# xhuan8/SoccerPlayerShapePose

Hardware: NVIDIA B200
Metric: SMPL meshes/sec fwd+bwd (higher is better)
Workload: dtype f32 (bf16x3 split on tcgen05, fp32 accumulate)

## Files before the change

### soccerplayershapepose_b200/build.py

```python
from __future__ import annotations

import concurrent.futures
import os
import shutil
import subprocess
import sys

HERE = os.path.dirname(os.path.abspath(__file__))
CSRC = os.path.join(HERE, "csrc")
BUILD = os.path.join(HERE, "csrc", "build")
LIB = os.path.join(HERE, "libb200smpl.so")

SOURCES = ["api.cu", "pack.cu", "pose.cu", "blend_simt.cu", "blend_umma.cu", "fused_fwd.cu", "lbs.cu", "joints.cu", "aux_ops.cu", "fit.cu", "loss.cu", "silhouette.cu"]
HEADERS = [os.path.join(CSRC, h) for h in sorted(os.listdir(CSRC)) if h.endswith(".cuh")] + [
    os.path.join(HERE, "..", "include", "b200smpl.h")]

NVCC_FLAGS = [
    "-gencode", "arch=compute_100a,code=sm_100a",
    "-O3", "-std=c++17", "-lineinfo",
    "-Xcompiler", "-fPIC",
    "-Xcompiler", "-fvisibility=hidden",
    "--expt-relaxed-constexpr",
    "-Xptxas", "-v",
]


def _nvcc() -> str:
    for cand in (os.environ.get("NVCC"), "/usr/local/cuda/bin/nvcc", shutil.which("nvcc")):
        if cand and os.path.exists(cand):
            return cand
    raise RuntimeError("nvcc not found (needed to build libb200smpl.so)")


def _stale(target: str, deps) -> bool:
    if not os.path.exists(target):
        return True
# ... 45 lines not shown
```

### soccerplayershapepose_b200/csrc/api.cu

```cuda
#include <atomic>
#include <cstring>
#include <map>
#include <mutex>

#include <nvtx3/nvToolsExt.h>

#include "common.cuh"
#include "umma_common.cuh"

namespace b200smpl {

bool pdl_enabled() {
  static const bool on = getenv("B200_PDL") == nullptr || atoi(getenv("B200_PDL")) != 0;
  return on;
}

NvtxRange::NvtxRange(const char* name) { nvtxRangePushA(name); }
NvtxRange::~NvtxRange() { nvtxRangePop(); }

static thread_local std::string g_last_error;
static std::atomic<long long> g_launches{0};

void set_error(const std::string& msg) { g_last_error = msg; }
int fail(int code, const std::string& msg) {
// ... 50 lines not shown
  const int S = slab_bodies > 0 ? round_up(std::min(slab_bodies, MAX_SLAB), 128) : DEFAULT_SLAB;
  p.S = std::min(S, Bp);
  size_t off = 0;
  auto take = [&](size_t bytes) {
    const size_t o = off;
    off = align_up(off + bytes, 1024);
    return o;
  };
  const size_t S_ = (size_t)p.S;
  p.off_feat = take(S_ * d.fl.pitch * 2);
  p.off_featf = take(mode == B200SMPL_MODE_FP32_SIMT ? S_ * d.fl.nf_pad * 4 : 0);
  p.off_A = take((size_t)NJ * AELEMS * S_ * 4);
  p.off_jposed = take((size_t)NJ * 3 * S_ * 4);
  p.off_vpT = take((size_t)d.n_pad * S_ * 4);
  p.saved_slab_bytes = align_up((size_t)NJ * AELEMS * S_ * 4, 1024) + align_up((size_t)d.n_pad * S_ * 4, 1024);
  if (backward) {
    const int bmode = bwd_gemm_mode(mode);
    p.k_splits = bmode == B200SMPL_MODE_FP32_SIMT ? 1 : blend_bwd_umma_splits(d, p.S, m->num_sms);
    p.off_dvp_hi = take(S_ * d.n_pad * 2);
    p.off_dvp_lo = take(bmode == B200SMPL_MODE_BF16 ? 0 : S_ * d.n_pad * 2);
    p.off_dA = take((size_t)(NJ * AELEMS + 3) * S_ * 4);
    p.off_dtr = p.off_dA + (size_t)NJ * AELEMS * S_ * 4;
    p.off_dJtot = take((size_t)std::max(batch, 1) * d.njout * 3 * 4);
    p.off_dfeat = take((size_t)p.k_splits * S_ * d.fl.nf_pad * 4);
  }
  p.total = off + 1024;
  return p;
}

static int check_common(const b200smpl_model* m, int batch, int mode, const void* ws) {
  if (m == nullptr) return fail(B200SMPL_ERR_INVALID, "null model handle");
  if (m->device < 0) return fail(B200SMPL_ERR_CUDA, "host-only model handle: no CUDA device (there is no CPU fallback)");
  if (batch < 1) return fail(B200SMPL_ERR_INVALID, "batch must be >= 1");
  if (mode != B200SMPL_MODE_FP32 && mode != B200SMPL_MODE_BF16 && mode != B200SMPL_MODE_FP32_SIMT &&
      mode != B200SMPL_MODE_BF16_FAST)
    return fail(B200SMPL_ERR_INVALID, "unknown mode");
  if (ws == nullptr) return fail(B200SMPL_ERR_WORKSPACE, "null workspace");
  return 0;
}

}

using namespace b200smpl;

extern "C" {

int b200smpl_abi_version(void) { return B200SMPL_ABI_VERSION; }
// ... 63 lines not shown
    m->num_sms = prop.multiProcessorCount;
    if (prop.major != 10) {
      cleanup();
      cudaSetDevice(prev);
      return fail(B200SMPL_ERR_CUDA, "this library is built for sm_100a (B200) only; device is sm_" +
                                         std::to_string(prop.major) + std::to_string(prop.minor));
    }
  }
  auto upload = [&](const void* src, size_t bytes, const void** dst) -> bool {
    void* p = nullptr;
    if (cudaMalloc(&p, std::max<size_t>(bytes, 16)) != cudaSuccess) return false;
    m->allocs.push_back(p);
    if (bytes && cudaMemcpy(p, src, bytes, cudaMemcpyHostToDevice) != cudaSuccess) return false;
    *dst = p;
    return true;
  };
  HostArrays& h = m->host;
  DevModel& d = m->dm;
  bool ok = true;
#define UP(field, vec) ok = ok && upload((vec).data(), (vec).size() * sizeof((vec)[0]), (const void**)&d.field)
  UP(Wf, h.Wf);
  UP(Wb_hi, h.Wb_hi);
  UP(Wb_lo, h.Wb_lo);
  UP(W32, h.W32);
  UP(vmeta, h.vmeta);
  UP(vwts, h.vwts);
  UP(vplan, h.vplan);
  UP(Jt, h.Jt);
  UP(Jsd, h.Jsd);
  UP(term_ptr, h.term_ptr);
  UP(term_joint, h.term_joint);
  UP(term_qrow, h.term_qrow);
  UP(term_c, h.term_c);
  UP(qmeta, h.qmeta);
  UP(qcoef, h.qcoef);
  UP(vt_j0, h.vt_j0);
  UP(vt_nj, h.vt_nj);
#undef UP
  cudaSetDevice(prev);
  if (!ok) {
    e = cudaGetLastError();
    cleanup();
    return fail(B200SMPL_ERR_CUDA, std::string("model upload failed: ") + cudaGetErrorString(e));
  }
  *out = m;
  return 0;
// ... 163 lines not shown
    const int nb = std::min(S, B - b0);
    const int Sw = round_up(nb, 128);
    B200_CUDA_TRY(cudaMemsetAsync(dA_part, 0, (size_t)(NJ * AELEMS + 3) * S * 4, st));
    if (saved) {
      A_T = (float*)(saved + (size_t)(b0 / S) * p.saved_slab_bytes);
      vpT = (float*)((char*)A_T + align_up((size_t)NJ * AELEMS * S * 4, 1024));
    } else {
      if ((rc = launch_pose_fwd(d, a->betas, a->pose, aa, b0, nb, S, Sw, feat, featf, A_T, nullptr, nullptr, st)))
        return rc;
      if (a->mode == B200SMPL_MODE_FP32_SIMT)
        rc = launch_blend_fwd_simt(d, featf, S, Sw, vpT, row_begin, d.n_pad, st);
      else
        rc = launch_blend_fwd_umma(d, fwd_gemm_mode(a->mode), feat, S, Sw, vpT, row_begin, d.n_pad, m->num_sms, st);
      if (rc) return rc;
    }
    {
      const size_t c0 = (size_t)row_end / 8, c1 = (size_t)round_up(row_end, 64) / 8;
      if (c1 > c0) {
        const size_t pitch = (size_t)(d.n_pad / 8) * 2048, width = (c1 - c0) * 2048;
        B200_CUDA_TRY(cudaMemset2DAsync(dvp_hi + c0 * 1024, pitch, 0, width, (size_t)Sw / 128, st));
        if (dvp_lo) B200_CUDA_TRY(cudaMemset2DAsync(dvp_lo + c0 * 1024, pitch, 0, width, (size_t)Sw / 128, st));
      }
    }
    if (have_v)
      if ((rc = launch_lbs_bwd(d, vpT, S, Sw, A_T, b0, nb, a->grad_vertices, dvp_hi, dvp_lo, dA_part, dtr_part,
                               m->num_sms, st)))
        return rc;
    if (have_j)
      if ((rc = launch_joints_bwd(d, vpT, S, Sw, A_T, b0, nb, dJ, dvp_hi, dvp_lo, dA_part, dtr_part, have_v, st))) return rc;
    if (a->mode == B200SMPL_MODE_FP32_SIMT)
      rc = launch_blend_bwd_simt(d, dvp_hi, dvp_lo, S, Sw, dfeat_part, row_begin, row_end, st);
    else
      rc = launch_blend_bwd_umma(d, bmode, dvp_hi, dvp_lo, S, Sw, dfeat_part, k_splits, row_begin, row_end, st);
    if (rc) return rc;
    if ((rc = launch_pose_bwd(d, a->betas, a->pose, aa, b0, nb, S, A_T, dA_part, 1, dtr_part, dfeat_part, k_splits,
                              have_j ? dJ : nullptr, a->grad_betas, a->grad_pose, a->grad_transl, st)))
      return rc;
  }
  return 0;
}

}
```

### soccerplayershapepose_b200/csrc/common.cuh

```cuda
#pragma once

#include <cuda_bf16.h>
#include <cuda_runtime.h>
#include <stdint.h>

#include <cstring>
#include <string>
#include <utility>
#include <vector>

#include "../../include/b200smpl.h"

namespace b200smpl {

constexpr int NJ = 24;
constexpr int NPOSE = 9 * (NJ - 1);
constexpr int AELEMS = 12;
constexpr int TILE_V = 32;
constexpr int MAX_CHILD = 4;
constexpr int MAX_BETAS = 16;

constexpr uint32_t VMETA_VALID = 1u << 29;

struct ChainTables {
// ... 34 lines not shown
  L.pitch = 64 + 2 * L.pseg;
  L.nf = nb + NPOSE;
  L.nf_pad = round_up(L.nf, 16);
  return L;
}

struct DevModel {
  int V;
  int ntiles;
  int n_real;
  int nq;
  int n_rows;
  int n_virt0;
  int n_pad;
  int njout;
  int nterms;
  int ntv;
  int vt_maxcols;
  FeatLayout fl;
  ChainTables chain;
  const __nv_bfloat16* Wf;
  const __nv_bfloat16* Wb_hi;
  const __nv_bfloat16* Wb_lo;
  const float* W32;
  const uint32_t* vmeta;
  const float4* vwts;
  const uint32_t* vplan;
  const float* Jt;
  const float* Jsd;
  const int32_t* term_ptr;
  const uint8_t* term_joint;
  const int32_t* term_qrow;
  const float* term_c;
  const uint32_t* qmeta;
  const float* qcoef;
  const int32_t* vt_j0;
  const int32_t* vt_nj;
};

struct HostArrays {
  std::vector<__nv_bfloat16> Wf, Wb_hi, Wb_lo;
  std::vector<float> W32, Jt, Jsd, term_c;
  std::vector<uint32_t> vmeta;
  std::vector<float> vwts;
  std::vector<uint32_t> vplan;
  std::vector<int32_t> term_ptr, term_qrow, vt_j0, vt_nj;
  std::vector<int8_t> chain_order, chain_level_ptr;
  std::vector<uint32_t> qmeta;
  std::vector<float> qcoef;
  std::vector<uint8_t> term_joint;
};

}

struct b200smpl_model {
  int device = -1;
  b200smpl::DevModel dm{};
  b200smpl::HostArrays host;
  std::vector<void*> allocs;
  int nvj = 0, nreg = 0;
  int num_sms = 148;
};

namespace b200smpl {
// ... 66 lines not shown
    ::b200smpl::count_launch();                                                                   \
  } while (0)

int pack_model(const b200smpl_model_desc* d, HostArrays& h, DevModel& dm, std::string& err);

int launch_pose_fwd(const DevModel& m, const float* betas, const float* pose, bool axis_angle, int b0, int nb, int S,
                    int Sw, __nv_bfloat16* feat, float* featf, float* A_blk, const float* transl, float* joints,
                    cudaStream_t st);
int launch_pose_bwd(const DevModel& m, const float* betas, const float* pose, bool axis_angle, int b0, int nb, int S,
                    const float* A_blk, const float* dA_part, int n_dA_parts, const float* dtr_part, const float* dfeat_part,
                    int n_dfeat_parts, const float* dJ, float* grad_betas, float* grad_pose,
                    float* grad_transl, cudaStream_t st);

int launch_blend_fwd_simt(const DevModel& m, const float* featf, int S, int Sw, float* vpT, int row_begin,
                          int row_end, cudaStream_t st);
int launch_blend_bwd_simt(const DevModel& m, const __nv_bfloat16* dvp_hi, const __nv_bfloat16* dvp_lo, int S, int Sw,
                          float* dfeat, int row_begin, int row_end, cudaStream_t st);
int launch_blend_fwd_umma(const DevModel& m, int mode, const __nv_bfloat16* feat, int S, int Sw, float* vpT,
                          int row_begin, int row_end, int num_sms, cudaStream_t st);
int launch_blend_bwd_umma(const DevModel& m, int mode, const __nv_bfloat16* dvp_hi, const __nv_bfloat16* dvp_lo,
                          int S, int Sw, float* dfeat_part, int nsplit, int row_begin, int row_end,
                          cudaStream_t st);
int blend_bwd_umma_splits(const DevModel& m, int S, int num_sms);
int launch_blend_lbs_fwd(const DevModel& m, int mode, const __nv_bfloat16* feat, int S, int Sw, float* vpT,
                         const float* A_blk, int b0, int nb, const float* transl, float* verts, int num_sms,
                         cudaStream_t st);

int launch_lbs_fwd(const DevModel& m, const float* vpT, int S, const float* A_T, int b0, int nb,
                   const float* transl, float* verts, int num_sms, cudaStream_t st);
int launch_lbs_bwd(const DevModel& m, const float* vpT, int S, int Sw, const float* A_T, int b0, int nb,
                   const float* grad_verts, __nv_bfloat16* dvp_hi, __nv_bfloat16* dvp_lo, float* dA_acc,
                   float* dtr_acc, int num_sms, cudaStream_t st);

int launch_joints_fwd(const DevModel& m, const float* vpB, int S, const float* A_blk, int b0, int nb,
                      const float* transl, float* joints, bool after_lbs, cudaStream_t st);
int launch_joints_bwd(const DevModel& m, const float* vpB, int S, int Sw, const float* A_blk, int b0, int nb,
                      const float* dJ, __nv_bfloat16* dvp_hi, __nv_bfloat16* dvp_lo, float* dA_part, float* dtr_part,
                      bool after_lbs, cudaStream_t st);
int launch_joint_grad_total(const float* joints, const float* cam, const float* gj, const float* g2d, float* dJ,
                            float* gcam, int B, int nj, cudaStream_t st);

}
```

### soccerplayershapepose_b200/csrc/lbs.cu

```cuda
#include "lbs_tiles.cuh"

namespace b200smpl {


struct CtaRange {
  int begin, end;
};
__device__ __forceinline__ CtaRange make_cta_range(int ngroups, int nitems) {
  const long long total = (long long)ngroups * nitems;
  CtaRange r;
  r.begin = (int)(total * blockIdx.x / gridDim.x);
  r.end = (int)(total * (blockIdx.x + 1) / gridDim.x);
  return r;
}

template <int HV>
__device__ __forceinline__ void issue_item(float4* vbuf, uint32_t* stash, uint64_t* bar, const float4* __restrict__ vp_group,
                                           const uint32_t* __restrict__ vplan, int t) {
  using SH = ItemShape<HV>;
  mbar_expect_tx(bar, SH::TX_BYTES);
  bulk_g2s(vbuf, vp_group + (size_t)t * (SH::NCH4 * 32), SH::VP_WORDS * 4, bar);
  bulk_g2s(stash, vplan + (size_t)t * SH::PLAN_WORDS, SH::PLAN_WORDS * 4, bar);
}
template <int HV>
__device__ __forceinline__ void global_to_tile_scalar(float* tile, const float* src0, size_t row_stride, int nrows,
                                                      int ncols, int lane) {
  for (int r = 0; r < 32; ++r)
    for (int c = lane; c < ItemShape<HV>::ROWS; c += 32)
      tile[r * ItemShape<HV>::HROW + c] = (r < nrows && c < ncols) ? src0[(size_t)r * row_stride + c] : 0.f;
}

constexpr int FWD_RUN = 1;
constexpr int FWD_HV = 16;
constexpr int FWD_WARPS = 8;
constexpr int FWD_THREADS = FWD_WARPS * 32;
constexpr int FWD_WARP_WORDS = ItemShape<FWD_HV>::TILE_WORDS + 2 * (ItemShape<FWD_HV>::VP_WORDS + ItemShape<FWD_HV>::PLAN_WORDS) + 4;
constexpr size_t FWD_SMEM = (size_t)(AG_WORDS + FWD_WARPS * FWD_WARP_WORDS) * 4 + 16;

template <bool HI>
__device__ __forceinline__ void load_slot2(SlotXY& s, SlotZ2& z, const float* A_s, int joint, int lane) {
  const float4* p = reinterpret_cast<const float4*>(A_s) + joint * 96 + lane;
  const float4 q0 = p[0], q1 = p[32], q2 = p[64];
  s.c0 = mk2(q0.x, q0.y); s.c1 = mk2(q0.z, q0.w); s.c2 = mk2(q1.x, q1.y); s.t = mk2(q1.z, q1.w);
  z.r20 = set_half<HI>(z.r20, q2.x); z.r21 = set_half<HI>(z.r21, q2.y);
  z.r22 = set_half<HI>(z.r22, q2.z); z.t2 = set_half<HI>(z.t2, q2.w);
}
// ... 347 lines not shown
```

### soccerplayershapepose_b200/csrc/lbs_tiles.cuh

```cuda
#pragma once

#include "skin_common.cuh"

namespace b200smpl {

template <int HV>
struct ItemShape {
  static constexpr int ROWS = HV * 3;
  static constexpr int HROW = ROWS + 4;
  static constexpr int TILE_WORDS = 32 * HROW;
  static constexpr int NCH4 = ROWS / 4;
  static constexpr int NCH8 = ROWS / 8;
  static constexpr int PAIRS = ROWS / 2;
  static constexpr int VP_WORDS = NCH4 * 128;
  static constexpr int PLAN_WORDS = (HV / 8) * 40;
  static constexpr uint32_t TX_BYTES = (VP_WORDS + PLAN_WORDS) * 4;
  static_assert((HROW / 4) % 2 == 1 && ROWS % 8 == 0 && HV % 8 == 0, "item shape");
};

__device__ __forceinline__ const float4* plan_wts(const uint32_t* stash, int u) {
  return reinterpret_cast<const float4*>(stash + (u >> 1) * 40 + (u & 1) * 16);
}
__device__ __forceinline__ const uint32_t* plan_meta(const uint32_t* stash, int u) {
  return stash + (u >> 1) * 40 + 32 + (u & 1) * 4;
}

template <int HV>
__device__ __forceinline__ void tile_to_global_full(const float* tile, float* dst0, size_t row_stride, int lane) {
  using SH = ItemShape<HV>;
  constexpr int RPP = 96 / SH::PAIRS, J = 32 / RPP;
  float* gp[3];
  const float* sp[3];
#pragma unroll
  for (int kk = 0; kk < 3; ++kk) {
    const int piece = kk * 32 + lane, rr = piece / SH::PAIRS, c = (piece - rr * SH::PAIRS) * 2;
    gp[kk] = dst0 + (size_t)rr * row_stride + c;
    sp[kk] = tile + rr * SH::HROW + c;
  }
  const size_t step = (size_t)RPP * row_stride;
#pragma unroll
  for (int j = 0; j < J; ++j)
#pragma unroll
// ... 120 lines not shown
```

### soccerplayershapepose_b200/csrc/pack.cu

```cuda
#include <algorithm>
#include <array>
#include <cmath>
#include <cstring>
#include <map>
#include <numeric>

#include "common.cuh"

namespace b200smpl {

static inline __nv_bfloat16 h_bf16(float x) { return __float2bfloat16_rn(x); }
static inline float h_f32(__nv_bfloat16 x) { return __bfloat162float(x); }

int pack_model(const b200smpl_model_desc* d, HostArrays& h, DevModel& dm, std::string& err) {
  const int V = d->num_verts, nb = d->num_betas, nvj = d->num_vertex_joints, nreg = d->num_regressed_joints;
  if (d->num_joints != NJ) { err = "num_joints must be 24"; return B200SMPL_ERR_INVALID; }
  if (V < 1 || V > (1 << 20)) { err = "bad num_verts"; return B200SMPL_ERR_INVALID; }
  if (nb < 1 || nb > MAX_BETAS) { err = "num_betas must be in [1,16]"; return B200SMPL_ERR_INVALID; }
  if (!d->v_template || !d->shapedirs || !d->posedirs || !d->J_regressor || !d->lbs_weights || !d->parents ||
      (nvj > 0 && !d->vertex_joint_ids) || (nreg > 0 && !d->joint_regressors)) {
    err = "null model array";
    return B200SMPL_ERR_INVALID;
  }
  const FeatLayout fl = make_feat_layout(nb);
// ... 163 lines not shown
  h.Wb_hi.assign((size_t)fl.nf_pad * n_pad, h_bf16(0.f));
  h.Wb_lo.assign((size_t)fl.nf_pad * n_pad, h_bf16(0.f));
  for (int n = 0; n < n_rows; ++n) {
    __nv_bfloat16* wr = h.Wf.data() + (size_t)n * fl.pitch;
    {
      const float t = h.W32[n];
      const __nv_bfloat16 t0 = h_bf16(t);
      const __nv_bfloat16 t1 = h_bf16(t - h_f32(t0));
      const __nv_bfloat16 t2 = h_bf16(t - h_f32(t0) - h_f32(t1));
      wr[0] = t0; wr[1] = t1; wr[2] = t2;
    }
    for (int f = 0; f < nf; ++f) {
      const float x = h.W32[(size_t)(1 + f) * n_pad + n];
      const __nv_bfloat16 hi = h_bf16(x), lo = h_bf16(x - h_f32(hi));
      if (f < nb) {
        wr[fl.off_s0 + f] = hi; wr[fl.off_s1 + f] = hi; wr[fl.off_s2 + f] = lo;
      } else {
        const int p = f - nb;
        wr[fl.off_p0 + p] = hi; wr[fl.off_p1 + p] = lo;
      }
      h.Wb_hi[(size_t)f * n_pad + n] = hi;
      h.Wb_lo[(size_t)f * n_pad + n] = lo;
    }
  }

  h.Jt.assign(NJ * 3, 0.f);
  h.Jsd.assign((size_t)NJ * 3 * nb, 0.f);
  for (int j = 0; j < NJ; ++j) {
    std::vector<double> acc(3 * (1 + nb), 0.0);
    for (int v = 0; v < V; ++v) {
      const double r = d->J_regressor[(size_t)j * V + v];
      if (r == 0.0) continue;
      for (int k = 0; k < 3; ++k) {
        acc[k * (1 + nb)] += r * (double)d->v_template[v * 3 + k];
        for (int l = 0; l < nb; ++l) acc[k * (1 + nb) + 1 + l] += r * (double)d->shapedirs[((size_t)v * 3 + k) * nb + l];
      }
    }
    for (int k = 0; k < 3; ++k) {
      h.Jt[j * 3 + k] = (float)acc[k * (1 + nb)];
      for (int l = 0; l < nb; ++l) h.Jsd[((size_t)j * 3 + k) * nb + l] = (float)acc[k * (1 + nb) + 1 + l];
    }
  }

  h.vmeta.assign((size_t)ntiles * TILE_V, 0u);
  h.vwts.assign((size_t)ntiles * TILE_V * 4, 0.f);
  {
// ... 76 lines not shown
```

Before: 6.913 million.

## Fuse LBS backward with blend-shape backward GEMM in a 2-CTA tcgen05 kernel

Adds a clustered 2-CTA kernel that computes the skinning backward (dA, dtrans) and writes the per-vertex position gradients straight into tensor memory as the A operand of a tcgen05 GEMM against a reinterleaved blend-weight matrix. This produces the dfeat partials without materializing dvp_hi/dvp_lo in global memory. The host gains a new interleaved weight layout and a work list, and the fused path only handles vertex gradients, so joint gradients still take the old blend backward path over the virtual rows. This trades two kernels and the global round trip of dvp for a heavier warp-specialized kernel with more partial slots to reduce.

```diff
diff --git a/soccerplayershapepose_b200/build.py b/soccerplayershapepose_b200/build.py
--- a/soccerplayershapepose_b200/build.py
+++ b/soccerplayershapepose_b200/build.py
@@ -11,7 +11,7 @@
 BUILD = os.path.join(HERE, "csrc", "build")
 LIB = os.path.join(HERE, "libb200smpl.so")
 
-SOURCES = ["api.cu", "pack.cu", "pose.cu", "blend_simt.cu", "blend_umma.cu", "fused_fwd.cu", "lbs.cu", "joints.cu", "aux_ops.cu", "fit.cu", "loss.cu", "silhouette.cu"]
+SOURCES = ["api.cu", "pack.cu", "pose.cu", "blend_simt.cu", "blend_umma.cu", "fused_fwd.cu", "fused_bwd.cu", "lbs.cu", "joints.cu", "aux_ops.cu", "fit.cu", "loss.cu", "silhouette.cu"]
 HEADERS = [os.path.join(CSRC, h) for h in sorted(os.listdir(CSRC)) if h.endswith(".cuh")] + [
     os.path.join(HERE, "..", "include", "b200smpl.h")]
 
diff --git a/soccerplayershapepose_b200/csrc/api.cu b/soccerplayershapepose_b200/csrc/api.cu
--- a/soccerplayershapepose_b200/csrc/api.cu
+++ b/soccerplayershapepose_b200/csrc/api.cu
@@ -96,7 +96,9 @@
     p.off_dA = take((size_t)(NJ * AELEMS + 3) * S_ * 4);
     p.off_dtr = p.off_dA + (size_t)NJ * AELEMS * S_ * 4;
     p.off_dJtot = take((size_t)std::max(batch, 1) * d.njout * 3 * 4);
-    p.off_dfeat = take((size_t)p.k_splits * S_ * d.fl.nf_pad * 4);
+    int parts = p.k_splits;
+    if (bmode != B200SMPL_MODE_FP32_SIMT) parts = std::max(0, fused_bwd_parts(d, p.S, m->num_sms)) + p.k_splits;
+    p.off_dfeat = take((size_t)parts * S_ * d.fl.nf_pad * 4);
   }
   p.total = off + 1024;
   return p;
@@ -206,6 +208,8 @@
   UP(Wf, h.Wf);
   UP(Wb_hi, h.Wb_hi);
   UP(Wb_lo, h.Wb_lo);
+  UP(Wbi_hi, h.Wbi_hi);
+  UP(Wbi_lo, h.Wbi_lo);
   UP(W32, h.W32);
   UP(vmeta, h.vmeta);
   UP(vwts, h.vwts);
@@ -415,18 +419,38 @@
         if (dvp_lo) B200_CUDA_TRY(cudaMemset2DAsync(dvp_lo + c0 * 1024, pitch, 0, width, (size_t)Sw / 128, st));
       }
     }
-    if (have_v)
-      if ((rc = launch_lbs_bwd(d, vpT, S, Sw, A_T, b0, nb, a->grad_vertices, dvp_hi, dvp_lo, dA_part, dtr_part,
-                               m->num_sms, st)))
+    int n_parts = k_splits;
+    if (have_v && fused_bwd_usable(d, a->mode, a->grad_vertices)) {
+      const int nfp = fused_bwd_parts(d, Sw, m->num_sms);
+      if (nfp < 0) return fail(B200SMPL_ERR_INVALID, "slab too wide for the fused backward work list");
+      B200_CUDA_TRY(cudaMemsetAsync(dfeat_part, 0, (size_t)nfp * S * d.fl.nf_pad * 4, st));
+      if ((rc = launch_lbs_bwd_gemm(d, bmode, vpT, S, Sw, A_T, b0, nb, a->grad_vertices, dA_part, dtr_part, dfeat_part,
+                                    m->num_sms, st)))
         return rc;
-    if (have_j)
-      if ((rc = launch_joints_bwd(d, vpT, S, Sw, A_T, b0, nb, dJ, dvp_hi, dvp_lo, dA_part, dtr_part, have_v, st))) return rc;
-    if (a->mode == B200SMPL_MODE_FP32_SIMT)
-      rc = launch_blend_bwd_simt(d, dvp_hi, dvp_lo, S, Sw, dfeat_part, row_begin, row_end, st);
-    else
-      rc = launch_blend_bwd_umma(d, bmode, dvp_hi, dvp_lo, S, Sw, dfeat_part, k_splits, row_begin, row_end, st);
-    if (rc) return rc;
-    if ((rc = launch_pose_bwd(d, a->betas, a->pose, aa, b0, nb, S, A_T, dA_part, 1, dtr_part, dfeat_part, k_splits,
+      n_parts = nfp;
+      if (have_j) {
+        if ((rc = launch_joints_bwd(d, vpT, S, Sw, A_T, b0, nb, dJ, dvp_hi, dvp_lo, dA_part, dtr_part, false, st))) return rc;
+        const int vslabs = (row_end + 63) / 64 - d.n_virt0 / 64;
+        const int ksv = std::max(1, std::min(p.k_splits, vslabs / MIN_SLABS_PER_SPLIT));
+        if ((rc = launch_blend_bwd_umma(d, bmode, dvp_hi, dvp_lo, S, Sw, dfeat_part + (size_t)nfp * S * d.fl.nf_pad, ksv,
+                                        d.n_virt0, row_end, st)))
+          return rc;
+        n_parts += ksv;
+      }
+    } else {
+      if (have_v)
+        if ((rc = launch_lbs_bwd(d, vpT, S, Sw, A_T, b0, nb, a->grad_vertices, dvp_hi, dvp_lo, dA_part, dtr_part,
+                                 m->num_sms, st)))
+          return rc;
+      if (have_j)
+        if ((rc = launch_joints_bwd(d, vpT, S, Sw, A_T, b0, nb, dJ, dvp_hi, dvp_lo, dA_part, dtr_part, have_v, st))) return rc;
+      if (a->mode == B200SMPL_MODE_FP32_SIMT)
+        rc = launch_blend_bwd_simt(d, dvp_hi, dvp_lo, S, Sw, dfeat_part, row_begin, row_end, st);
+      else
+        rc = launch_blend_bwd_umma(d, bmode, dvp_hi, dvp_lo, S, Sw, dfeat_part, k_splits, row_begin, row_end, st);
+      if (rc) return rc;
+    }
+    if ((rc = launch_pose_bwd(d, a->betas, a->pose, aa, b0, nb, S, A_T, dA_part, 1, dtr_part, dfeat_part, n_parts,
                               have_j ? dJ : nullptr, a->grad_betas, a->grad_pose, a->grad_transl, st)))
       return rc;
   }
diff --git a/soccerplayershapepose_b200/csrc/common.cuh b/soccerplayershapepose_b200/csrc/common.cuh
--- a/soccerplayershapepose_b200/csrc/common.cuh
+++ b/soccerplayershapepose_b200/csrc/common.cuh
@@ -80,6 +80,8 @@
   const __nv_bfloat16* Wf;
   const __nv_bfloat16* Wb_hi;
   const __nv_bfloat16* Wb_lo;
+  const __nv_bfloat16* Wbi_hi;
+  const __nv_bfloat16* Wbi_lo;
   const float* W32;
   const uint32_t* vmeta;
   const float4* vwts;
@@ -97,7 +99,7 @@
 };
 
 struct HostArrays {
-  std::vector<__nv_bfloat16> Wf, Wb_hi, Wb_lo;
+  std::vector<__nv_bfloat16> Wf, Wb_hi, Wb_lo, Wbi_hi, Wbi_lo;
   std::vector<float> W32, Jt, Jsd, term_c;
   std::vector<uint32_t> vmeta;
   std::vector<float> vwts;
@@ -210,6 +212,11 @@
                           int S, int Sw, float* dfeat_part, int nsplit, int row_begin, int row_end,
                           cudaStream_t st);
 int blend_bwd_umma_splits(const DevModel& m, int S, int num_sms);
+bool fused_bwd_usable(const DevModel& m, int mode, const float* grad_verts);
+int fused_bwd_parts(const DevModel& m, int Sw, int num_sms);
+int launch_lbs_bwd_gemm(const DevModel& m, int mode, const float* vpB, int S, int Sw, const float* A_blk, int b0, int nb,
+                        const float* grad_verts, float* dA_acc, float* dtr_acc, float* dfeat_part, int num_sms,
+                        cudaStream_t st);
 int launch_blend_lbs_fwd(const DevModel& m, int mode, const __nv_bfloat16* feat, int S, int Sw, float* vpT,
                          const float* A_blk, int b0, int nb, const float* transl, float* verts, int num_sms,
                          cudaStream_t st);
diff --git a/soccerplayershapepose_b200/csrc/fused_bwd.cu b/soccerplayershapepose_b200/csrc/fused_bwd.cu
--- /dev/null
+++ b/soccerplayershapepose_b200/csrc/fused_bwd.cu
@@ -0,0 +1,509 @@
+#include <algorithm>
+
+#include "lbs_tiles.cuh"
+#include "umma_common.cuh"
+
+namespace b200smpl {
+
+constexpr int FB_BN_MAX = 224;
+constexpr int FB_ITEM_V = 16;
+constexpr int FB_ITEM_ROWS = 3 * FB_ITEM_V;
+constexpr int FB_ROT_COL0 = FB_BN_MAX;
+constexpr int FB_ROT_COLS = 8;
+constexpr int FB_NSTAGE_A = 2;
+constexpr int FB_A_COL0 = FB_ROT_COL0 + NJ * FB_ROT_COLS;
+constexpr int FB_A_STAGE_COLS = FB_ITEM_ROWS;
+constexpr int FB_NSTAGE_B = 2;
+constexpr int FB_BSTAGE_MAX = 2 * (FB_ITEM_ROWS / 8) * (FB_BN_MAX / 2) * 16;
+constexpr int FB_PROD_WARPS = 8;
+constexpr int FB_PROD_WARP0 = 4;
+constexpr int FB_THREADS = (FB_PROD_WARP0 + FB_PROD_WARPS) * 32;
+constexpr int FB_REGS_WG0 = 56;
+constexpr int FB_REGS_PROD = 224;
+constexpr int FB_HV = 8;
+using FbShape = ItemShape<FB_HV>;
+constexpr int FB_R22_WORDS = 4 * NJ * 32;
+constexpr int FB_WARP_BYTES = (2 * FbShape::TILE_WORDS + 2 * (FbShape::VP_WORDS + FbShape::PLAN_WORDS)) * 4;
+constexpr int FB_NBARS = 2 * FB_NSTAGE_A + 3 * FB_NSTAGE_B + 1 + 2 * FB_PROD_WARPS;
+constexpr size_t FB_SMEM = (size_t)FB_NSTAGE_B * FB_BSTAGE_MAX + (size_t)FB_R22_WORDS * 4 + (size_t)FB_PROD_WARPS * FB_WARP_BYTES +
+                           FB_NBARS * 8 + 16 + 1024 ;
+static_assert(FB_SMEM + 1024 <= 164 * 1024, "fused backward: above the 164 KB carve-out the dV pieces lose L1");
+static_assert(FB_A_COL0 + FB_NSTAGE_A * FB_A_STAGE_COLS <= 512, "fused backward: tensor memory budget");
+static_assert(FB_REGS_WG0 * 128 + FB_REGS_PROD * 256 <= 65536, "register file");
+static_assert(FB_WARP_BYTES % 16 == 0, "bulk-copy destinations stay 16-byte aligned");
+
+struct FbWork {
+  uint16_t bp[BS_MAX_WORK], i0[BS_MAX_WORK], i1[BS_MAX_WORK], slot[BS_MAX_WORK];
+};
+
+__device__ __forceinline__ void umma_bf16_2cta_ts(uint32_t tmem_d, uint32_t tmem_a, uint64_t desc_b, uint32_t idesc,
+                                                  uint32_t accumulate) {
+  asm volatile(
+      "{\n\t.reg .pred p;\n\t"
+      "setp.ne.b32 p, %4, 0;\n\t"
+      "tcgen05.mma.cta_group::2.kind::f16 [%0], [%1], %2, %3, p;\n\t}"
+      ::"r"(tmem_d), "r"(tmem_a), "l"(desc_b), "r"(idesc), "r"(accumulate)
+      : "memory");
+}
+__device__ __forceinline__ void tmem_st_x4u(uint32_t taddr, uint32_t a, uint32_t b, uint32_t c, uint32_t d) {
+  asm volatile("tcgen05.st.sync.aligned.32x32b.x4.b32 [%0], {%1, %2, %3, %4};" ::"r"(taddr), "r"(a), "r"(b), "r"(c), "r"(d)
+               : "memory");
+}
+__device__ __forceinline__ void tmem_ld_x8(uint32_t taddr, uint32_t (&r)[8]) {
+  asm volatile(
+      "tcgen05.ld.sync.aligned.32x32b.x8.b32 {%0, %1, %2, %3, %4, %5, %6, %7}, [%8];\n\t"
+      "tcgen05.wait::ld.sync.aligned;"
+      : "=r"(r[0]), "=r"(r[1]), "=r"(r[2]), "=r"(r[3]), "=r"(r[4]), "=r"(r[5]), "=r"(r[6]), "=r"(r[7])
+      : "r"(taddr)
+      : "memory");
+}
+
+template <bool HI>
+__device__ __forceinline__ void load_rot_half_t(SlotPair& P, float& r22, uint32_t trot, const float* r22_g, int joint, int lane) {
+  uint32_t r[8];
+  tmem_ld_x8(trot + (uint32_t)(joint * FB_ROT_COLS), r);
+  P.R[0] = set_half<HI>(P.R[0], __uint_as_float(r[0])); P.R[3] = set_half<HI>(P.R[3], __uint_as_float(r[1]));
+  P.R[1] = set_half<HI>(P.R[1], __uint_as_float(r[2])); P.R[4] = set_half<HI>(P.R[4], __uint_as_float(r[3]));
+  P.R[2] = set_half<HI>(P.R[2], __uint_as_float(r[4])); P.R[5] = set_half<HI>(P.R[5], __uint_as_float(r[5]));
+  P.R[6] = set_half<HI>(P.R[6], __uint_as_float(r[6])); P.R[7] = set_half<HI>(P.R[7], __uint_as_float(r[7]));
+  r22 = r22_g[joint * 32 + lane];
+}
+
+__device__ __forceinline__ void tmem_ld_x8_nowait(uint32_t taddr, uint32_t (&r)[8]) {
+  asm volatile("tcgen05.ld.sync.aligned.32x32b.x8.b32 {%0, %1, %2, %3, %4, %5, %6, %7}, [%8];"
+               : "=r"(r[0]), "=r"(r[1]), "=r"(r[2]), "=r"(r[3]), "=r"(r[4]), "=r"(r[5]), "=r"(r[6]), "=r"(r[7])
+               : "r"(taddr)
+               : "memory");
+}
+template <bool HI>
+__device__ __forceinline__ void set_rot_half(SlotPair& P, float& r22, uint32_t (&r)[8], const float* r22_g, int joint, int lane) {
+#pragma unroll
+  for (int i = 0; i < 8; ++i) asm volatile("" : "+r"(r[i]));
+  P.R[0] = set_half<HI>(P.R[0], __uint_as_float(r[0])); P.R[3] = set_half<HI>(P.R[3], __uint_as_float(r[1]));
+  P.R[1] = set_half<HI>(P.R[1], __uint_as_float(r[2])); P.R[4] = set_half<HI>(P.R[4], __uint_as_float(r[3]));
+  P.R[2] = set_half<HI>(P.R[2], __uint_as_float(r[4])); P.R[5] = set_half<HI>(P.R[5], __uint_as_float(r[5]));
+  P.R[6] = set_half<HI>(P.R[6], __uint_as_float(r[6])); P.R[7] = set_half<HI>(P.R[7], __uint_as_float(r[7]));
+  r22 = r22_g[joint * 32 + lane];
+}
+
+__device__ __forceinline__ void skin_bwd4_t(BwdState& s, float (&z22)[4], uint32_t trot, const float* r22_g,
+                                            float* __restrict__ dA_g, int lane, const uint32_t* meta_s, const float4* wts_s,
+                                            uint32_t force, const float4* vp_s, const float* row_in, float (&G)[12]) {
+  const uint4 m4 = *reinterpret_cast<const uint4*>(meta_s);
+  const uint32_t mts[4] = {m4.x | force, m4.y, m4.z, m4.w};
+  float P[12];
+#pragma unroll
+  for (int i = 0; i < 3; ++i) {
+    const float4 v = vp_s[i * 32];
+    P[i * 4] = v.x; P[i * 4 + 1] = v.y; P[i * 4 + 2] = v.z; P[i * 4 + 3] = v.w;
+    const float4 h = *reinterpret_cast<const float4*>(row_in + i * 4);
+    G[i * 4] = h.x; G[i * 4 + 1] = h.y; G[i * 4 + 2] = h.z; G[i * 4 + 3] = h.w;
+  }
+  float4 w = wts_s[0];
+#pragma unroll
+  for (int i = 0; i < 4; ++i) {
+    const uint32_t mt = mts[i];
+    const float4 wn = wts_s[i < 3 ? i + 1 : 3];
+    if (mt & (0xFu << 20)) {
+      const uint32_t pv = s.prev;
+#ifdef FB_BATCH_LD
+      uint32_t r[4][8];
+#pragma unroll
+      for (int k = 0; k < 4; ++k)
+        if (mt & (1u << (20 + k))) tmem_ld_x8_nowait(trot + (uint32_t)(((mt >> (5 * k)) & 31) * FB_ROT_COLS), r[k]);
+      if (mt & (1u << 20)) flush_half<false>(s.A, dA_g, pv & 31, lane);
+      if (mt & (1u << 21)) flush_half<true>(s.A, dA_g, (pv >> 5) & 31, lane);
+      if (mt & (1u << 22)) flush_half<false>(s.B, dA_g, (pv >> 10) & 31, lane);
+      if (mt & (1u << 23)) flush_half<true>(s.B, dA_g, (pv >> 15) & 31, lane);
+      asm volatile("tcgen05.wait::ld.sync.aligned;" ::: "memory");
+      if (mt & (1u << 20)) set_rot_half<false>(s.A, z22[0], r[0], r22_g, mt & 31, lane);
+      if (mt & (1u << 21)) set_rot_half<true>(s.A, z22[1], r[1], r22_g, (mt >> 5) & 31, lane);
+      if (mt & (1u << 22)) set_rot_half<false>(s.B, z22[2], r[2], r22_g, (mt >> 10) & 31, lane);
+      if (mt & (1u << 23)) set_rot_half<true>(s.B, z22[3], r[3], r22_g, (mt >> 15) & 31, lane);
+#else
+      if (mt & (1u << 20)) { flush_half<false>(s.A, dA_g, pv & 31, lane); load_rot_half_t<false>(s.A, z22[0], trot, r22_g, mt & 31, lane); }
+      if (mt & (1u << 21)) { flush_half<true>(s.A, dA_g, (pv >> 5) & 31, lane); load_rot_half_t<true>(s.A, z22[1], trot, r22_g, (mt >> 5) & 31, lane); }
+      if (mt & (1u << 22)) { flush_half<false>(s.B, dA_g, (pv >> 10) & 31, lane); load_rot_half_t<false>(s.B, z22[2], trot, r22_g, (mt >> 10) & 31, lane); }
+      if (mt & (1u << 23)) { flush_half<true>(s.B, dA_g, (pv >> 15) & 31, lane); load_rot_half_t<true>(s.B, z22[3], trot, r22_g, (mt >> 15) & 31, lane); }
+#endif
+    }
+    s.prev = mt;
+    const f2 px = bc2(P[i * 3]), py = bc2(P[i * 3 + 1]), pz = bc2(P[i * 3 + 2]);
+    const float gx = G[i * 3], gy = G[i * 3 + 1], gz = G[i * 3 + 2];
+    s.sx += gx; s.sy += gy; s.sz += gz;
+    const f2 wA = mk2(w.x, w.y), wB = mk2(w.z, w.w);
+    const f2 hxA = mul2(wA, bc2(gx)), hyA = mul2(wA, bc2(gy)), hzA = mul2(wA, bc2(gz));
+    const f2 hxB = mul2(wB, bc2(gx)), hyB = mul2(wB, bc2(gy)), hzB = mul2(wB, bc2(gz));
+    f2 qx = fma2(s.A.R[0], hxA, fma2(s.A.R[3], hyA, mul2(s.A.R[6], hzA)));
+    f2 qy = fma2(s.A.R[1], hxA, fma2(s.A.R[4], hyA, mul2(s.A.R[7], hzA)));
+    f2 qz = fma2(s.A.R[2], hxA, fma2(s.A.R[5], hyA, mul2(mk2(z22[0], z22[1]), hzA)));
+    qx = fma2(s.B.R[0], hxB, fma2(s.B.R[3], hyB, fma2(s.B.R[6], hzB, qx)));
+    qy = fma2(s.B.R[1], hxB, fma2(s.B.R[4], hyB, fma2(s.B.R[7], hzB, qy)));
+    qz = fma2(s.B.R[2], hxB, fma2(s.B.R[5], hyB, fma2(mk2(z22[2], z22[3]), hzB, qz)));
+    G[i * 3] = lo2(qx) + hi2(qx); G[i * 3 + 1] = lo2(qy) + hi2(qy); G[i * 3 + 2] = lo2(qz) + hi2(qz);
+#define B200_ACC(P_, hx_, hy_, hz_)                                                                  \
+  P_.D[0] = fma2(hx_, px, P_.D[0]); P_.D[1] = fma2(hx_, py, P_.D[1]); P_.D[2] = fma2(hx_, pz, P_.D[2]);   \
+  P_.D[3] = add2(P_.D[3], hx_);                                                                      \
+  P_.D[4] = fma2(hy_, px, P_.D[4]); P_.D[5] = fma2(hy_, py, P_.D[5]); P_.D[6] = fma2(hy_, pz, P_.D[6]);   \
+  P_.D[7] = add2(P_.D[7], hy_);                                                                      \
+  P_.D[8] = fma2(hz_, px, P_.D[8]); P_.D[9] = fma2(hz_, py, P_.D[9]); P_.D[10] = fma2(hz_, pz, P_.D[10]); \
+  P_.D[11] = add2(P_.D[11], hz_);
+    B200_ACC(s.A, hxA, hyA, hzA)
+    B200_ACC(s.B, hxB, hyB, hzB)
+#undef B200_ACC
+    w = wn;
+  }
+}
+
+__device__ __forceinline__ void fb_arrive(uint64_t* bar, uint32_t rank) {
+  if (rank == 0) asm volatile("mbarrier.arrive.shared::cta.b64 _, [%0];" ::"r"(smem_u32(bar)) : "memory");
+  else remote_arrive(bar, 0);
+}
+
+__device__ __forceinline__ int fb_item_of_stage(int k, int i0, int n) {
+  return i0 + ((k & 1) ? (n + 1) / 2 + (k >> 1) : (k >> 1));
+}
+
+template <int BN, bool SPLIT3>
+__global__ void __launch_bounds__(FB_THREADS, 1)
+lbs_bwd_gemm_kernel(const float4* __restrict__ vpB, int nc4, const float4* __restrict__ A_blk, int b0, int nb,
+                    int ntiles_n, const float* __restrict__ grad_verts, int V, const uint32_t* __restrict__ vplan,
+                    const __nv_bfloat16* __restrict__ Wbi_hi, const __nv_bfloat16* __restrict__ Wbi_lo, int nitems_all,
+                    const __grid_constant__ FbWork work, float* __restrict__ dA_acc, float* __restrict__ dtr_acc,
+                    float* __restrict__ D, long long part_stride) {
+  constexpr uint32_t TMEM_COLS = 512;
+  constexpr int BNH = BN / 2;
+  constexpr int BCHUNK = BNH * 16;
+  constexpr int BTILE = (FB_ITEM_ROWS / 8) * BCHUNK;
+  using SH = FbShape;
+  extern __shared__ __align__(1024) unsigned char smem_dyn[];
+  unsigned char* smem = smem_dyn + ((1024u - (smem_u32(smem_dyn) & 1023u)) & 1023u);
+  unsigned char* b_s = smem;
+  float* r22_s = reinterpret_cast<float*>(b_s + FB_NSTAGE_B * FB_BSTAGE_MAX);
+  unsigned char* warp_s = reinterpret_cast<unsigned char*>(r22_s + FB_R22_WORDS);
+  uint64_t* bars = reinterpret_cast<uint64_t*>(warp_s + FB_PROD_WARPS * FB_WARP_BYTES);
+  uint64_t* a_full = bars;
+  uint64_t* a_empty = a_full + FB_NSTAGE_A;
+  uint64_t* b_full = a_empty + FB_NSTAGE_A;
+  uint64_t* peer_b_full = b_full + FB_NSTAGE_B;
+  uint64_t* b_empty = peer_b_full + FB_NSTAGE_B;
+  uint64_t* tmem_full = b_empty + FB_NSTAGE_B;
+  uint64_t* wbars = tmem_full + 1;
+  uint32_t* tmem_slot = reinterpret_cast<uint32_t*>(wbars + 2 * FB_PROD_WARPS);
+
+  const int warp = threadIdx.x >> 5, lane = threadIdx.x & 31;
+  const uint32_t rank = cluster_ctarank();
+  const int piece = (int)(blockIdx.x >> 1);
+  const int btile = (int)work.bp[piece] * 2 + (int)rank;
+  const int i0 = work.i0[piece], nit = (int)work.i1[piece] - i0;
+
+  if (warp == 1 && lane == 0) {
+    for (int i = 0; i < FB_NSTAGE_A; ++i) {
+      mbar_init(&a_full[i], 8);
+      mbar_init(&a_empty[i], 1);
+    }
+    for (int i = 0; i < FB_NSTAGE_B; ++i) {
+      mbar_init(&b_full[i], 1);
+      mbar_init(&peer_b_full[i], 1);
+      mbar_init(&b_empty[i], 1);
+    }
+    mbar_init(tmem_full, 1);
+    for (int i = 0; i < 2 * FB_PROD_WARPS; ++i) mbar_init(&wbars[i], 1);
+    fence_barrier_init();
+  }
+  if (warp == 1) {
+    __syncwarp();
+    asm volatile("tcgen05.alloc.cta_group::2.sync.aligned.shared::cta.b32 [%0], %1;" ::"r"(smem_u32(tmem_slot)), "r"(TMEM_COLS)
+                 : "memory");
+    asm volatile("tcgen05.relinquish_alloc_permit.cta_group::2.sync.aligned;" ::: "memory");
+  }
+  tc_fence_before();
+  cluster_sync_all();
+  tc_fence_after();
+  const uint32_t tmem_base = *tmem_slot;
+
+  if (warp < FB_PROD_WARP0) {
+    asm volatile("setmaxnreg.dec.sync.aligned.u32 %0;" ::"n"(FB_REGS_WG0));
+#ifndef FB_PRODUCERS_ONLY
+    if (warp == 0) {
+      const uint64_t pol_keep = l2_policy_evict_last();
+      int sb = 0;
+      uint32_t phase = 0;
+      for (int k = 0; k < nit; ++k) {
+        const int item = fb_item_of_stage(k, i0, nit);
+        mbar_wait(&b_empty[sb], phase ^ 1);
+        if (elect_one()) {
+          mbar_arrive_expect_tx(&b_full[sb], SPLIT3 ? 2 * BTILE : BTILE);
+          const size_t off = ((size_t)rank * nitems_all + item) * (BTILE / 2);
+          bulk_g2s_hint(b_s + sb * FB_BSTAGE_MAX, Wbi_hi + off, BTILE, &b_full[sb], pol_keep);
+          if (SPLIT3) bulk_g2s_hint(b_s + sb * FB_BSTAGE_MAX + BTILE, Wbi_lo + off, BTILE, &b_full[sb], pol_keep);
+        }
+        __syncwarp();
+        if (++sb == FB_NSTAGE_B) { sb = 0; phase ^= 1; }
+      }
+    } else if (warp == 1) {
+      int sb = 0;
+      uint32_t bphase = 0;
+      if (rank == 0) {
+        constexpr uint32_t idesc = make_idesc(2 * BM, BN);
+        const uint64_t db_base = make_nosw_desc(smem_u32(b_s), BCHUNK, 128);
+        for (int k = 0; k < nit; ++k) {
+          const int sa = k % FB_NSTAGE_A;
+          mbar_wait(&a_full[sa], (uint32_t)(k / FB_NSTAGE_A) & 1u);
+          mbar_wait(&b_full[sb], bphase);
+          mbar_wait(&peer_b_full[sb], bphase);
+          tc_fence_after();
+          const uint32_t a_hi = tmem_base + (uint32_t)(FB_A_COL0 + sa * FB_A_STAGE_COLS);
+          const uint32_t a_lo = a_hi + FB_A_STAGE_COLS / 2;
+          const uint64_t b_hi = db_base + (uint64_t)((sb * FB_BSTAGE_MAX) >> 4), b_lo = b_hi + (uint64_t)(BTILE >> 4);
+          if (elect_one()) {
+#pragma unroll
+            for (int ks = 0; ks < FB_ITEM_ROWS / UMMA_K; ++ks) {
+              const uint64_t bo = (uint64_t)((ks * 2 * BCHUNK) >> 4);
+              umma_bf16_2cta_ts(tmem_base, a_hi + ks * 8, b_hi + bo, idesc, (k | ks) != 0);
+              if (SPLIT3) {
+                umma_bf16_2cta_ts(tmem_base, a_lo + ks * 8, b_hi + bo, idesc, 1u);
+                umma_bf16_2cta_ts(tmem_base, a_hi + ks * 8, b_lo + bo, idesc, 1u);
+              }
+            }
+            umma_commit_2cta(&a_empty[sa]);
+            umma_commit_2cta(&b_empty[sb]);
+            if (k == nit - 1) umma_commit_2cta(tmem_full);
+          }
+          __syncwarp();
+          if (++sb == FB_NSTAGE_B) { sb = 0; bphase ^= 1; }
+        }
+      } else {
+        for (int k = 0; k < nit; ++k) {
+          mbar_wait(&b_full[sb], bphase);
+          if (elect_one()) remote_arrive(&peer_b_full[sb], 0);
+          __syncwarp();
+          if (++sb == FB_NSTAGE_B) { sb = 0; bphase ^= 1; }
+        }
+      }
+    }
+#else
+    if (warp == 1 && rank == 0) {
+      for (int k = 0; k < nit; ++k) {
+        const int sa = k % FB_NSTAGE_A;
+        mbar_wait(&a_full[sa], (uint32_t)(k / FB_NSTAGE_A) & 1u);
+        if (elect_one()) {
+          asm volatile("mbarrier.arrive.shared::cta.b64 _, [%0];" ::"r"(smem_u32(&a_empty[sa])) : "memory");
+          remote_arrive(&a_empty[sa], 1);
+          if (k == nit - 1) {
+            asm volatile("mbarrier.arrive.shared::cta.b64 _, [%0];" ::"r"(smem_u32(tmem_full)) : "memory");
+            remote_arrive(tmem_full, 1);
+          }
+        }
+        __syncwarp();
+      }
+    }
+#endif
+  } else {
+    asm volatile("setmaxnreg.inc.sync.aligned.u32 %0;" ::"n"(FB_REGS_PROD));
+    int lane_p = lane, q_p = warp & 3, h_p = (warp - FB_PROD_WARP0) >> 2;
+    asm volatile("" : "+r"(lane_p), "+r"(q_p), "+r"(h_p));
+    const int lane = lane_p, q = q_p, h = h_p, e = h * 4 + q;
+    const bool live = btile < ntiles_n;
+    const int g = btile * 4 + q;
+    float* r22_g = r22_s + q * NJ * 32;
+    unsigned char* wb = warp_s + e * FB_WARP_BYTES;
+    float* tiles = reinterpret_cast<float*>(wb);
+    float4* vbufs = reinterpret_cast<float4*>(wb + 2 * SH::TILE_WORDS * 4);
+    uint32_t* stash = reinterpret_cast<uint32_t*>(wb + (2 * SH::TILE_WORDS + 2 * SH::VP_WORDS) * 4);
+    uint64_t* wbar = wbars + e * 2;
+    const uint32_t lane_base = tmem_base + ((uint32_t)(q * 32) << 16);
+    const uint32_t trot = lane_base + FB_ROT_COL0;
+    if (live) {
+      const float4* ap = A_blk + (size_t)g * (NJ * 3 * 32) + lane;
+#pragma unroll 1
+      for (int j = h * (NJ / 2); j < (h + 1) * (NJ / 2); ++j) {
+        const float4 x0 = ap[(j * 3) * 32], x1 = ap[(j * 3 + 1) * 32], x2 = ap[(j * 3 + 2) * 32];
+        tmem_st_x4u(trot + j * FB_ROT_COLS, __float_as_uint(x0.x), __float_as_uint(x0.y), __float_as_uint(x0.z), __float_as_uint(x0.w));
+        tmem_st_x4u(trot + j * FB_ROT_COLS + 4, __float_as_uint(x1.x), __float_as_uint(x1.y), __float_as_uint(x2.x), __float_as_uint(x2.y));
+        r22_g[j * 32 + lane] = x2.z;
+      }
+      asm volatile("tcgen05.wait::st.sync.aligned;" ::: "memory");
+    }
+    tc_fence_before();
+    asm volatile("bar.sync %0, %1;" ::"r"(1 + q), "n"(64) : "memory");
+    tc_fence_after();
+    const int n_first = (nit + 1) / 2;
+    const int my_n = h == 0 ? n_first : nit - n_first;
+    const int it_first = i0 + (h == 0 ? 0 : n_first);
+    const int nrows = max(0, min(32, nb - g * 32));
+    const size_t row_stride = (size_t)V * 3;
+    const uint32_t a_col = lane_base + (uint32_t)(FB_A_COL0 + h * FB_A_STAGE_COLS);
+    if (live && my_n > 0) {
+      float* dA_g = dA_acc + (size_t)g * AG_WORDS;
+      const float4* vp_g = vpB + (size_t)g * nc4 * 32;
+      const float* dv_g = grad_verts + (size_t)(b0 + g * 32) * V * 3;
+      const int t8_first = it_first * 2, t8_end = (it_first + my_n) * 2;
+      if (lane == 0) issue_item<FB_HV>(vbufs, stash, &wbar[0], vp_g, vplan, t8_first);
+      issue_rows<FB_HV>(tiles, dv_g + (size_t)t8_first * FB_HV * 3, row_stride, nrows, max(0, min(FB_HV, V - t8_first * FB_HV)) * 3, lane);
+      cp_async_commit();
+      BwdState st;
+#pragma unroll
+      for (int i = 0; i < AELEMS; ++i) st.A.D[i] = st.B.D[i] = mk2(0.f, 0.f);
+#pragma unroll
+      for (int i = 0; i < 9; ++i) st.A.R[i] = st.B.R[i] = mk2(0.f, 0.f);
+      st.prev = 0u;
+      st.sx = st.sy = st.sz = 0.f;
+      float z22[4] = {0.f, 0.f, 0.f, 0.f};
+      uint32_t n_used = 0;
+#pragma unroll 1
+      for (int m = 0; m < my_n; ++m) {
+#pragma unroll 1
+        for (int hh = 0; hh < 2; ++hh, ++n_used) {
+          const int t8 = t8_first + 2 * m + hh;
+          const uint32_t b = n_used & 1;
+          if (t8 + 1 < t8_end) {
+            if (lane == 0)
+              issue_item<FB_HV>(vbufs + (b ^ 1) * (SH::NCH4 * 32), stash + (b ^ 1) * SH::PLAN_WORDS, &wbar[b ^ 1], vp_g, vplan, t8 + 1);
+            issue_rows<FB_HV>(tiles + (b ^ 1) * SH::TILE_WORDS, dv_g + (size_t)(t8 + 1) * FB_HV * 3, row_stride, nrows,
+                              max(0, min(FB_HV, V - (t8 + 1) * FB_HV)) * 3, lane);
+          }
+          cp_async_commit();
+          cp_async_wait<1>();
+          __syncwarp();
+          mbar_wait(&wbar[b], (n_used >> 1) & 1);
+          const float4* vp_s = vbufs + b * (SH::NCH4 * 32) + lane;
+          const uint32_t* ps = stash + b * SH::PLAN_WORDS;
+          const float* my_row = tiles + b * SH::TILE_WORDS + lane * SH::HROW;
+          uint32_t hi[12], lo[12];
+#pragma unroll
+          for (int u = 0; u < 2; ++u) {
+            float G[12];
+            skin_bwd4_t(st, z22, trot, r22_g, dA_g, lane, plan_meta(ps, u), plan_wts(ps, u),
+                        (m == 0 && hh == 0 && u == 0) ? (0xFu << 20) : 0u, vp_s + u * 96, my_row + u * 12, G);
+#pragma unroll
+            for (int c = 0; c < 6; ++c) split2(G[2 * c], G[2 * c + 1], hi[u * 6 + c], lo[u * 6 + c]);
+          }
+          if (hh == 0) {
+            mbar_wait(&a_empty[h], ((uint32_t)m & 1u) ^ 1u);
+            tc_fence_after();
+          }
+#pragma unroll
+          for (int c = 0; c < 12; c += 4) {
+            tmem_st_x4u(a_col + hh * 12 + c, hi[c], hi[c + 1], hi[c + 2], hi[c + 3]);
+            if (SPLIT3) tmem_st_x4u(a_col + FB_A_STAGE_COLS / 2 + hh * 12 + c, lo[c], lo[c + 1], lo[c + 2], lo[c + 3]);
+          }
+          __syncwarp();
+        }
+        asm volatile("tcgen05.wait::st.sync.aligned;" ::: "memory");
+        tc_fence_before();
+        __syncwarp();
+        if (lane == 0) fb_arrive(&a_full[h], rank);
+      }
+      bwd_close_group(st, dA_g, dtr_acc + (size_t)g * 96, lane);
+    } else {
+      for (int m = 0; m < my_n; ++m) {
+        mbar_wait(&a_empty[h], ((uint32_t)m & 1u) ^ 1u);
+        __syncwarp();
+        if (lane == 0) fb_arrive(&a_full[h], rank);
+      }
+    }
+    if (nit > 0) {
+      mbar_wait(tmem_full, 0);
+      tc_fence_after();
+      if (live) {
+        float* drow = D + (long long)work.slot[piece] * part_stride + (long long)(btile * BM + q * 32 + lane) * BN + h * BNH;
+#pragma unroll 1
+        for (int c0 = 0; c0 < BNH; c0 += 8) {
+          uint32_t v[8];
+          tmem_ld_x8(lane_base + (uint32_t)(h * BNH + c0), v);
+          *reinterpret_cast<uint4*>(drow + c0) = make_uint4(v[0], v[1], v[2], v[3]);
+          *reinterpret_cast<uint4*>(drow + c0 + 4) = make_uint4(v[4], v[5], v[6], v[7]);
+        }
+      }
+    }
+  }
+  tc_fence_before();
+  cluster_sync_all();
+  if (warp == 1) {
+    tc_fence_after();
+    asm volatile("tcgen05.dealloc.cta_group::2.sync.aligned.b32 %0, %1;" ::"r"(tmem_base), "r"(TMEM_COLS) : "memory");
+  }
+}
+
+static int fb_build_work(const DevModel& m, int Sw, int num_sms, FbWork& work, int& npieces) {
+  BsWork bs;
+  const int bp_total = (Sw / BM + 1) / 2;
+  npieces = build_bs_work(bp_total, m.ntiles * (TILE_V / FB_ITEM_V), std::max(1, num_sms / 2), bs);
+  if (npieces < 0) return -1;
+  int nslots = 0;
+  std::vector<int> used(bp_total, 0);
+  memset(&work, 0, sizeof(work));
+  for (int c = 0; c < npieces; ++c) {
+    work.bp[c] = bs.bp[c]; work.i0[c] = bs.w0[c]; work.i1[c] = bs.w1[c];
+    work.slot[c] = (uint16_t)used[bs.bp[c]]++;
+    nslots = std::max(nslots, (int)work.slot[c] + 1);
+  }
+  return nslots;
+}
+
+bool fused_bwd_usable(const DevModel& m, int mode, const float* grad_verts) {
+  return mode != B200SMPL_MODE_FP32_SIMT && (m.fl.nf_pad == 208 || m.fl.nf_pad == 224) && (m.V & 1) == 0 &&
+         (reinterpret_cast<uintptr_t>(grad_verts) & 7) == 0 && m.n_virt0 == m.ntiles * 96;
+}
+
+int fused_bwd_parts(const DevModel& m, int Sw, int num_sms) {
+  FbWork work;
+  int npieces = 0;
+  return fb_build_work(m, Sw, num_sms, work, npieces);
+}
+
+template <int BN, bool SPLIT3>
+static cudaError_t fb_launch(const cudaLaunchConfig_t& cfg, const DevModel& m, const float* vpB, const float* A_blk, int b0,
+                             int nb, int Sw, const float* grad_verts, const FbWork& work, float* dA_acc, float* dtr_acc,
+                             float* dfeat_part, int S) {
+  static bool attr_done[64] = {};
+  int dev = 0;
+  cudaError_t e = cudaGetDevice(&dev);
+  if (e != cudaSuccess) return e;
+  if (dev < 0 || dev >= 64 || !attr_done[dev]) {
+    e = cudaFuncSetAttribute(lbs_bwd_gemm_kernel<BN, SPLIT3>, cudaFuncAttributeMaxDynamicSharedMemorySize, (int)FB_SMEM);
+    if (e != cudaSuccess) return e;
+    if (dev >= 0 && dev < 64) attr_done[dev] = true;
+  }
+  return cudaLaunchKernelEx(&cfg, lbs_bwd_gemm_kernel<BN, SPLIT3>, reinterpret_cast<const float4*>(vpB), m.n_pad / 4,
+                            reinterpret_cast<const float4*>(A_blk), b0, nb, Sw / BM, grad_verts, m.V, m.vplan, m.Wbi_hi,
+                            m.Wbi_lo, m.ntiles * (TILE_V / FB_ITEM_V), work, dA_acc, dtr_acc, dfeat_part,
+                            (long long)S * BN);
+}
+
+int launch_lbs_bwd_gemm(const DevModel& m, int mode, const float* vpB, int S, int Sw, const float* A_blk, int b0, int nb,
+                        const float* grad_verts, float* dA_acc, float* dtr_acc, float* dfeat_part, int num_sms,
+                        cudaStream_t st) {
+  FbWork work;
+  int npieces = 0;
+  const int nslots = fb_build_work(m, Sw, num_sms, work, npieces);
+  if (nslots < 0) return fail(B200SMPL_ERR_INVALID, "slab too wide for the fused backward work list");
+  const bool split3 = mode != B200SMPL_MODE_BF16;
+  cudaLaunchConfig_t cfg;
+  memset(&cfg, 0, sizeof(cfg));
+  cfg.gridDim = dim3(2 * npieces, 1, 1);
+  cfg.blockDim = dim3(FB_THREADS, 1, 1);
+  cfg.dynamicSmemBytes = FB_SMEM;
+  cfg.stream = st;
+  cudaLaunchAttribute attr[1];
+  attr[0].id = cudaLaunchAttributeClusterDimension;
+  attr[0].val.clusterDim.x = 2;
+  attr[0].val.clusterDim.y = 1;
+  attr[0].val.clusterDim.z = 1;
+  cfg.attrs = attr;
+  cfg.numAttrs = 1;
+  LaunchTimer _timer("lbs_bwd_gemm", st);
+  cudaError_t e;
+  if (m.fl.nf_pad == 224)
+    e = split3 ? fb_launch<224, true>(cfg, m, vpB, A_blk, b0, nb, Sw, grad_verts, work, dA_acc, dtr_acc, dfeat_part, S)
+               : fb_launch<224, false>(cfg, m, vpB, A_blk, b0, nb, Sw, grad_verts, work, dA_acc, dtr_acc, dfeat_part, S);
+  else
+    e = split3 ? fb_launch<208, true>(cfg, m, vpB, A_blk, b0, nb, Sw, grad_verts, work, dA_acc, dtr_acc, dfeat_part, S)
+               : fb_launch<208, false>(cfg, m, vpB, A_blk, b0, nb, Sw, grad_verts, work, dA_acc, dtr_acc, dfeat_part, S);
+  if (e != cudaSuccess) return fail(B200SMPL_ERR_CUDA, std::string("lbs_bwd_gemm: ") + cudaGetErrorString(e));
+  B200_LAUNCH_CHECK("lbs_bwd_gemm");
+  return 0;
+}
+
+}
diff --git a/soccerplayershapepose_b200/csrc/lbs.cu b/soccerplayershapepose_b200/csrc/lbs.cu
--- a/soccerplayershapepose_b200/csrc/lbs.cu
+++ b/soccerplayershapepose_b200/csrc/lbs.cu
@@ -14,14 +14,6 @@
   return r;
 }
 
-template <int HV>
-__device__ __forceinline__ void issue_item(float4* vbuf, uint32_t* stash, uint64_t* bar, const float4* __restrict__ vp_group,
-                                           const uint32_t* __restrict__ vplan, int t) {
-  using SH = ItemShape<HV>;
-  mbar_expect_tx(bar, SH::TX_BYTES);
-  bulk_g2s(vbuf, vp_group + (size_t)t * (SH::NCH4 * 32), SH::VP_WORDS * 4, bar);
-  bulk_g2s(stash, vplan + (size_t)t * SH::PLAN_WORDS, SH::PLAN_WORDS * 4, bar);
-}
 template <int HV>
 __device__ __forceinline__ void global_to_tile_scalar(float* tile, const float* src0, size_t row_stride, int nrows,
                                                       int ncols, int lane) {
diff --git a/soccerplayershapepose_b200/csrc/lbs_tiles.cuh b/soccerplayershapepose_b200/csrc/lbs_tiles.cuh
--- a/soccerplayershapepose_b200/csrc/lbs_tiles.cuh
+++ b/soccerplayershapepose_b200/csrc/lbs_tiles.cuh
@@ -18,6 +18,14 @@
   static_assert((HROW / 4) % 2 == 1 && ROWS % 8 == 0 && HV % 8 == 0, "item shape");
 };
 
+template <int HV>
+__device__ __forceinline__ void issue_item(float4* vbuf, uint32_t* stash, uint64_t* bar, const float4* __restrict__ vp_group,
+                                           const uint32_t* __restrict__ vplan, int t) {
+  using SH = ItemShape<HV>;
+  mbar_expect_tx(bar, SH::TX_BYTES);
+  bulk_g2s(vbuf, vp_group + (size_t)t * (SH::NCH4 * 32), SH::VP_WORDS * 4, bar);
+  bulk_g2s(stash, vplan + (size_t)t * SH::PLAN_WORDS, SH::PLAN_WORDS * 4, bar);
+}
 __device__ __forceinline__ const float4* plan_wts(const uint32_t* stash, int u) {
   return reinterpret_cast<const float4*>(stash + (u >> 1) * 40 + (u & 1) * 16);
 }
diff --git a/soccerplayershapepose_b200/csrc/pack.cu b/soccerplayershapepose_b200/csrc/pack.cu
--- a/soccerplayershapepose_b200/csrc/pack.cu
+++ b/soccerplayershapepose_b200/csrc/pack.cu
@@ -209,6 +209,21 @@
       h.Wb_hi[(size_t)f * n_pad + n] = hi;
       h.Wb_lo[(size_t)f * n_pad + n] = lo;
     }
+  }
+  {
+    const int nh = fl.nf_pad / 2, nitems = ntiles * 2;
+    h.Wbi_hi.assign((size_t)2 * nitems * 6 * nh * 8, h_bf16(0.f));
+    h.Wbi_lo.assign((size_t)2 * nitems * 6 * nh * 8, h_bf16(0.f));
+    for (int half = 0; half < 2; ++half)
+      for (int it = 0; it < nitems; ++it)
+        for (int c = 0; c < 6; ++c)
+          for (int f = 0; f < nh; ++f)
+            for (int r = 0; r < 8; ++r) {
+              const size_t src = (size_t)(half * nh + f) * n_pad + (size_t)it * 48 + c * 8 + r;
+              const size_t dst = ((((size_t)half * nitems + it) * 6 + c) * nh + f) * 8 + r;
+              h.Wbi_hi[dst] = h.Wb_hi[src];
+              h.Wbi_lo[dst] = h.Wb_lo[src];
+            }
   }
 
   h.Jt.assign(NJ * 3, 0.f);
```

Measured after the change: 6.938 million, median of 6. No clear change (+0.4%).
